# eniac/otti

Hardware: AMD Instinct MI355X
Metric: R1CS constraints/sec proved (Spartan NIZK) at 2^20 (higher is better)
Workload: dtype u256 (GF(l) / GF(2^255-19), 8 x u32 limbs)

## Files before the change

otti_amd/csrc/device.h:

```cpp
#pragma once
#include <hip/hip_runtime.h>
#include <vector>
#include <functional>
#include <cstddef>
#include <chrono>
#include "spartan.h"
#include "mail.h"
#include "msm_plan.h"

namespace otti {

#define OTTI_HIP(expr) ::otti::hip_check((expr), #expr, __FILE__, __LINE__)
void hip_check(hipError_t e, const char *what, const char *file, int line);
struct OutOfDeviceMemory : Error { using Error::Error; };
struct TailTimeout : Error { using Error::Error; };

template <class T> struct DevBuf {
    T *p = nullptr; size_t n = 0;
    DevBuf() {}
    explicit DevBuf(size_t count) { alloc(count); }
    DevBuf(const DevBuf &) = delete; DevBuf &operator=(const DevBuf &) = delete;
    DevBuf(DevBuf &&o) noexcept : p(o.p), n(o.n) { o.p = nullptr; o.n = 0; }
    DevBuf &operator=(DevBuf &&o) noexcept { if (this != &o) { release(); p = o.p; n = o.n; o.p = nullptr; o.n = 0; } return *this; }
    ~DevBuf() { release(); }
    void alloc(size_t count) { release(); if (count) OTTI_HIP(hipMalloc((void **)&p, count * sizeof(T))); n = count; }
    void release() { if (p) (void)hipFree(p); p = nullptr; n = 0; }
};

struct DCsr3 { const uint32_t *ptr[3]; const uint32_t *idx[3]; const Fr *val[3]; const int32_t *small[3]; };
struct DeviceCsrSet {
    DevBuf<uint32_t> ptr[3], idx[3]; DevBuf<Fr> val[3];
    DevBuf<int32_t> small[3];
    bool use_small = false;
    DevBuf<uint32_t> heavy;
    DevBuf<uint32_t> seg_row, seg_no, seg_begin;
    size_t rows = 0, n_heavy = 0, n_seg = 0;
    double avg_row = 0.0;
    bool quad() const { return avg_row >= 3.0; }
    DCsr3 view() const { DCsr3 v; for (int k = 0; k < 3; k++) { v.ptr[k] = ptr[k].p; v.idx[k] = idx[k].p; v.val[k] = val[k].p; v.small[k] = small[k].p; } return v; }
};
struct DeviceInstance { DeviceCsrSet by_row, by_col; size_t nnz = 0; };
struct DeviceShard { int rank = 0, world = 1; DeviceCsrSet by_row, by_col; };

struct DeviceGens {
    DevBuf<TabEntry> table; int c = 0, W = 0; size_t E = 0, nbases = 0;
    double build_ms[2] = {0, 0};
    const TabEntry *entry0(size_t base) const { return table.p + base * (size_t)W * E; }
};

struct Mailbox { Fr *partials; unsigned *counter; Fr *host_results; unsigned long long *host_flag; unsigned long long seq; int slot; int line_mail = 0;
                 Fr *dev_results; };

struct alignas(64) GoBox { unsigned long long seq, tag, pad[2]; Fr v[4]; unsigned long long timed_out, pad2[3]; };
static_assert(sizeof(GoBox) == 192 && offsetof(GoBox, v) == 32 && offsetof(GoBox, timed_out) == 160, "GoBox layout is read by hand-written loads");
constexpr int kGoCopies = 8;
constexpr size_t kGoCopyStride = 4096;
constexpr int kMsmMailRegions = 4;
struct PtFe;
bool msm_mail_sum(const MsmMail *m, int i0, int i1, unsigned long long want, PtFe &acc, unsigned max_spins, bool allow_ifma);
bool msm_mails_whole(const MsmMail *m, int n, unsigned long long want);
struct MsmPending { unsigned long long seq = 0, order = 0; int region = 0; uint32_t rows = 0, nchunks = 0; };
struct DevCtx;
struct MsmMailbox {
    MsmMail *host = nullptr, *dev = nullptr;
    MsmPending pending[kMsmMailRegions]; int pending_n = 0;
    unsigned long long launches = 0;
    unsigned long long read[8] = {0}; int read_next = 0;
    unsigned long long order = 0, h_pts_order = 0;
    bool host_sum(const DevCtx &c) const;
    void ensure(DevCtx &c);
    void queue(unsigned long long seq, uint32_t rows, uint32_t nchunks);
    MsmMail *region(int r) const { return host + (size_t)r * kMsmMailCap; }
};
struct TailMailbox { TailMail *host = nullptr, *dev = nullptr; void ensure(DevCtx &c); };
struct WaitLimits;
struct Armed { GoBox *host; GoBox *dev; unsigned long long want, deadline; int relay = 1, pollers = 1; };
constexpr unsigned long long kArmDeadlineTicks = 3000000000ull;
constexpr int kMaxBlocks = 2048;
constexpr size_t kArmMaxLen = 65536;

struct DevCtx {
    hipStream_t stream = nullptr;
    hipStream_t side = nullptr; hipEvent_t ev_side = nullptr;
    hipStream_t side_stream();
    int device = 0, num_cu = 256;
    DevBuf<Fr> partials;
    DevBuf<Fr> spmv_partial;
    DevBuf<Fr> results;
    Fr *h_results = nullptr;
    Fr *d_results_alias = nullptr;
    unsigned long long *h_flag = nullptr, *d_flag_alias = nullptr, seq = 0;
    DevBuf<unsigned> d_counter;
    DevBuf<unsigned long long> d_counts;
    DevBuf<unsigned long long> sat_bits;
    DevBuf<uint32_t> sat_rows; DevBuf<Fr> sat_abc;
    DevBuf<unsigned long long> diff_chunks;
    Mailbox next_mailbox(int slot);
    GoBox *h_go = nullptr, *d_go_alias = nullptr; DevBuf<GoBox> d_go; unsigned long long go_issued = 0, go_published = 0;
    unsigned long long arm_deadline = kArmDeadlineTicks;
    bool host_coherent = false;
    void reset_arrival_counters();
    hipEvent_t ev_order = nullptr;
    std::vector<struct RowSumSlot *> row_slots;
    TailMailbox tail_mail;
    template <class Pred, class OnLimit> void spin_until(Pred arrived, const WaitLimits &lim, std::chrono::steady_clock::time_point t0, OnLimit fail);
    void wait_tail(int n_groups, unsigned long long seq);
    void wait_tail_sums(int n_inst, int W, unsigned long long seq, Fr *sums);
    Armed arm_many(int count);
    bool armed_ok() const;
    Armed arm();
    void go(const Fr *v, int n);
    void go_abort();
    void wait_ticket(unsigned long long ticket);
    DevBuf<Pt> msm_keep;
    DevBuf<Pt> msm_partial, msm_final;
    Pt *h_pts = nullptr;
    size_t pending_host_encode = 0;
    uint8_t *h_points = nullptr;
    uint8_t *d_points_host = nullptr;
    DevBuf<uint8_t> d_points;
    size_t msm_partial_cap = 0, points_cap = 0;
    hipEvent_t ev0 = nullptr, ev1 = nullptr;
    static DevCtx &get();
    DevCtx() {} DevCtx(const DevCtx &) = delete; DevCtx &operator=(const DevCtx &) = delete;
    struct Scratch *scratch = nullptr;
    struct SnarkScratch *snark_scratch = nullptr;
    void sync();
    void wait_points(const MsmTicket &ticket);
    void encode_pending();
    Pt *d_pts_alias = nullptr; DevBuf<unsigned> d_counter2;
    MsmMailbox msm_mail;
    void msm_host_sum(const MsmPending &p);
    void ensure_points(size_t rows, size_t splits);
};
struct RowSumSlot { DevBuf<uint8_t> comp; DevBuf<Niels> pts; DevBuf<Fr> sc; DevBuf<Pt> out; DevBuf<unsigned> bad; bool busy = false; };
hipStream_t bulk_masked_stream();
struct ActiveProof { ActiveProof(); ~ActiveProof(); static int count(); };
constexpr int kResultSlots = 8192;

enum KClass { KC_MSM_ROWS = 0, KC_MSM_SMALL, KC_MSM_FINISH, KC_SC_CUBIC, KC_SC_QUAD, KC_SPMV, KC_EQ, KC_REDUCE, KC_BOUND, KC_BULLET, KC_OTHER,
              KC_PC_ROUND, KC_PROD_LAYER, KC_HASH_LAYER, KC_GATHER, KC_DOT_MANY ,
              KC_DECODE, KC_MSM_VAR , KC_SAT_CHECK , KC_COUNT };
struct KStats {
    bool on = false; unsigned mask = 0xffffffffu;
    std::vector<hipEvent_t> pool; std::vector<int> cls; size_t used = 0;
    double total_ms[KC_COUNT] = {0}; unsigned long long count[KC_COUNT] = {0};
    static KStats &get();
    int begin(DevCtx &c, int k);
    void end(DevCtx &c, int rec);
    void flush();
    void reset();
};
struct KScope { DevCtx &c; int rec; KScope(DevCtx &c_, int k) : c(c_), rec(KStats::get().begin(c_, k)) {} ~KScope() { KStats::get().end(c, rec); } };

enum WitFormat { WIT_CANONICAL32 = 0, WIT_MONTGOMERY32 = 1, WIT_I64 = 2, WIT_U64 = 3 };
inline size_t wit_elem_bytes(int format) { return format == WIT_I64 || format == WIT_U64 ? 8 : 32; }
struct DeviceWitness {
    DevBuf<Fr> z; std::vector<Fr> inputs;
    double small_fraction = 0.0;
    DeviceWitness(const Instance &I, int format, const void *src, size_t nvars, size_t stride, bool src_on_device, hipStream_t producer, const std::vector<Fr> &inputs);
    DeviceWitness(const Instance &I, const uint8_t *vars32, size_t nvars, const std::vector<Fr> &inputs) : DeviceWitness(I, WIT_CANONICAL32, vars32, nvars, 0, false, nullptr, inputs) {}
    void update(size_t first, int format, const void *src, size_t count, size_t stride, bool src_on_device, hipStream_t producer);
    void scatter(const uint64_t *idx, int format, const void *src, size_t count, size_t stride, bool on_device, hipStream_t producer);
    unsigned long long scatter_calls = 0, rows_patched = 0, terms_patched = 0;
    size_t assign(size_t first, int format, const void *src, size_t count, size_t stride, bool src_on_device, hipStream_t producer);
    size_t diff(size_t first, int format, const void *src, size_t count, size_t stride, bool src_on_device, hipStream_t producer, uint64_t *idx_out, size_t cap) const;
    unsigned long long assign_calls = 0, assign_changed = 0, assign_resums = 0;
    void set_inputs(const std::vector<Fr> &new_inputs);
    DevBuf<Pt> rows_kept; const char *rows_stream = nullptr; size_t rows_R = 0;
    Gens *rows_gens = nullptr;
    unsigned long long rows_resummed = 0;
    bool rows_kept_for(const Gens &g) const;
    void keep_rows(Gens &g);
    void drop_rows();
private:
    std::vector<Fr> set_up(DevCtx &c, const Instance &I, size_t nvars);
};
void ensure_device_objects(Instance &I, Gens &g);
void ensure_instance_device(Instance &I);
void ensure_gens_device(Gens &g);
void release_gens_device(Gens &g);
int device_window_bits(size_t nbases);
constexpr int kInstEvalSlot = 16;
void instance_evaluate_begin(Instance &I, const std::vector<Fr> &rx, const std::vector<Fr> &ry);
void instance_evaluate_finish(Fr out[3]);
void instance_evaluate_gpu(Instance &I, const std::vector<Fr> &rx, const std::vector<Fr> &ry, Fr out[3]);
class ShardComm;
std::vector<uint8_t> nizk_prove_resident(Instance &I, DeviceWitness &wit, Gens &g, const void *tlabel, size_t tlabel_len, const uint8_t *seed32,
                                         ProveTimings *tm, ShardComm *sh = nullptr);
struct R1csHooks { std::function<void(const std::vector<Fr> &)> on_rx, on_ry; std::function<void()> on_idle; };
void r1cs_prove_device(Instance &I, DeviceWitness &wit, Gens &g, Transcript &tr, RandomTape &tape, NizkProof &P, ProveTimings &T, ShardComm *sh, const R1csHooks *hooks = nullptr);
std::shared_ptr<DeviceShard> upload_instance_shard(const Instance &I, int rank, int world);
struct PeBufs { Fr *LZ, *Rv, *a, *s, *b2, *s2, *rows, *extras; };
DotProductProofLog dplog_prove_device(DevCtx &c, const DeviceGens &DG, const Gens &g, const PcView &v, const PeBufs &B, const Fr &LZ_blind, const Fr *y_known,
                                      const Fr &blind_y, CPoint &Cy_out, Transcript &tr, RandomTape &tape);
size_t dev_witness_ingest_from(DevCtx &c, int format, const void *src, size_t stride, size_t n, Fr *z, size_t dst_off, size_t *n_small = nullptr);
void dev_witness_scatter_check(DevCtx &c, int format, const void *src, size_t stride, const uint64_t *d_idx, size_t n, size_t V, Fr *conv,
                               size_t *bad_scalars, size_t *bad_indices);
void dev_witness_scatter_apply(DevCtx &c, const uint64_t *d_idx, const Fr *conv, size_t n, size_t V, Fr *z, Fr *delta);
struct WitDiff { size_t n_changed = 0, bad_scalars = 0, lo = 0, hi = 0; };
size_t dev_witness_diff_chunk();
WitDiff dev_witness_diff_count(DevCtx &c, int format, const void *src, size_t stride, size_t n, const Fr *z);
void dev_witness_diff_apply(DevCtx &c, int format, const void *src, size_t stride, size_t n, Fr *z, size_t first, size_t cap, uint64_t *d_idx, Fr *delta, bool write_z);
void dev_witness_rows_touched(DevCtx &c, const uint64_t *d_idx, size_t n, size_t R, uint64_t *h_rows);
void dev_gather_strided(DevCtx &c, const Fr *in, size_t stride, size_t offset, Fr *out, size_t n);

std::shared_ptr<DeviceInstance> upload_instance(const Instance &I);
std::shared_ptr<DeviceGens> build_device_gens(const Gens &g, int window_bits);

void dev_fr_op(DevCtx &c, int op, const Fr *a, const Fr *b, Fr *out, size_t n);
void dev_from_canonical(DevCtx &c, const Fr *in, Fr *out, size_t n);
void dev_to_canonical(DevCtx &c, const Fr *in, Fr *out, size_t n);
void dev_fill_zero(DevCtx &c, Fr *p, size_t n);
void dev_spmv3(DevCtx &c, const DeviceCsrSet &m, const Fr *x, Fr *out0, Fr *out1, Fr *out2, bool combine, const Fr coef[3]);
constexpr int kSatCountSlot = 24;
constexpr size_t kSatReportRows = 64;
struct SatReport { uint64_t n_unsat = 0; std::vector<uint64_t> rows; std::vector<uint8_t> abc96; float kernel_ms = 0; };
void dev_sat_pass(DevCtx &c, const DeviceCsrSet &m, const Fr *z, unsigned long long *bits);
uint64_t dev_sat_count(DevCtx &c);
SatReport dev_check_sat(DevCtx &c, DeviceInstance &d, const Fr *z, size_t max_rows, bool with_values);
void dev_eq_evals(DevCtx &c, const Fr *r_host, size_t ell, Fr *out, Fr *scratch );
void dev_eq_evals2(DevCtx &c, const Fr *r0_host, size_t ell0, Fr *out0, const Fr *r1_host, size_t ell1, Fr *out1, Fr *scratch);
unsigned long long dev_sc_cubic_eval(DevCtx &c, const Fr *A, const Fr *B, const Fr *C, const Fr *D, size_t len, int slot);
unsigned long long dev_sc_cubic_fold_eval(DevCtx &c, Fr *A, Fr *B, Fr *C, Fr *D, size_t len, const Fr &r, int slot);
struct EqSrc { const Fr *hi, *lo; int lo_bits;
               uint32_t stride = 1, offset = 0;
               int top_bit = -1; Fr top; };
void dev_eq_pyramid(DevCtx &c, const Fr *r_host, size_t n, Fr *out );
void dev_eq_pyramid2(DevCtx &c, const Fr *r0_host, size_t n0, Fr *out0, const Fr *r1_host, size_t n1, Fr *out1);
unsigned long long dev_sc_cubic3_eval(DevCtx &c, const Fr *B, const Fr *C, const Fr *D, size_t len, const EqSrc &E, int slot);
unsigned long long dev_sc_cubic3_fold_eval(DevCtx &c, Fr *B, Fr *C, Fr *D, size_t len, const Fr &r, const EqSrc &E, int slot);
unsigned long long dev_sc_cubic3_fold_eval_armed(DevCtx &c, Fr *B, Fr *C, Fr *D, size_t len, const EqSrc &E, int slot);
unsigned long long dev_sc_quad_fold_eval_armed(DevCtx &c, Fr *A, Fr *B, size_t len, int slot);
unsigned long long dev_sc_quad_eval(DevCtx &c, const Fr *A, const Fr *B, size_t len, int slot);
unsigned long long dev_sc_quad_fold_eval(DevCtx &c, Fr *A, Fr *B, size_t len, const Fr &r, int slot);
void dev_fold_top(DevCtx &c, Fr *Z, size_t len, const Fr &r);
void dev_fold_bot(DevCtx &c, const Fr *Z, Fr *out, size_t len, const Fr &r);
void dev_fetch(DevCtx &c, const Fr *src, int slot, size_t n);
struct MsmJob {
    const Fr *dense = nullptr; size_t n_dense = 0, rows = 0;
    const Fr *extra_s = nullptr; const uint32_t *extra_base = nullptr ; size_t n_extra = 0;
    int mode = MSM_COMPRESSED;
    const Pt *addend = nullptr;
    bool sparse = false;
    Pt *keep_dst = nullptr; bool force_bulk = false;
};
constexpr double kSparseWitness = 0.25;
MsmTicket dev_msm_rows(DevCtx &c, const DeviceGens &g, const MsmJob &job);
double dev_small_fraction(DevCtx &c, const Fr *z, size_t n);
void dev_msm_scatter(DevCtx &c, const DeviceGens &g, const uint64_t *d_idx, const Fr *d_s, size_t count, size_t R, Pt *rows, size_t L);
void dev_encode_points(DevCtx &c, const Pt *pts, size_t n, uint8_t *d_out32);
void dev_poly_bound(DevCtx &c, const Fr *Z, size_t L, size_t R, const Fr *Lv, Fr *out, Fr *scratch );
bool dev_poly_bound_chunks(DevCtx &c, const Fr *Z, size_t L, size_t R, const Fr *Lv_rest, size_t m, Fr *out, Fr *scratch );
void dev_dot(DevCtx &c, const Fr *a, const Fr *b, size_t n, int slot);
void dev_bullet_step(DevCtx &c, Fr *a, Fr *b, Fr *s, size_t R, size_t n_cur, bool fold_first, const Fr &u, const Fr &u_inv, Fr *rows, Fr *extra_out);
void dev_bullet_finish(DevCtx &c, Fr *a, Fr *b, Fr *s, size_t R, const Fr &u, const Fr &u_inv, const Fr &d, Fr *rows, int slot_a);
struct BulletRound {
    size_t R, n_cur; bool fold; Fr u, u_inv;
    const Fr *a_in, *b_in, *s_in; Fr *a_out, *b_out, *s_out;
    const Fr *extra_s; const uint32_t *extra_base; bool armed = false;
};
MsmTicket dev_bullet_round(DevCtx &c, const DeviceGens &g, const BulletRound &round);
void dev_decode_niels(DevCtx &c, const uint8_t *compressed_dev, size_t n, Niels *out, unsigned *bad);
int dev_msm_var(DevCtx &c, const Niels *pts, const Fr *scalars, size_t n, Pt *out, size_t out_cap, int *n_windows, int *n_splits);
double dev_madd_peak(DevCtx &c);
void dev_fr_to_lanes(hipStream_t st, const Fr *d_src, const Fr *factor, unsigned long long *d_lanes, size_t n);
double dev_fr_mul_peak(DevCtx &c);
void dev_scale(DevCtx &c, const Fr *in, const Fr &k, Fr *out, size_t n);
void dev_fill_one(DevCtx &c, Fr *p, size_t n);

}
```

otti_amd/csrc/k_sumcheck.hip:

```cpp
#include "kernels_common.h"

namespace otti {

struct FrArgs { Fr v[13]; };
struct EqJob { FrArgs r; int n; int pyramid; Fr *out; };
constexpr int kEqLow = 6, kEqTreeBlock = 256, kEqTreeGroups = 16;
__device__ __forceinline__ Fr eq_mul9(const Fr &x, const Fr &y) { return fr9_pack_lt2l(fr9_mul(fr9_unpack5(x), fr9_unpack(y))); }
__global__ __launch_bounds__(kEqTreeBlock) void k_eq_tree(EqJob j0, EqJob j1) {
    const EqJob &J = blockIdx.y ? j1 : j0;
    const int n = J.n, a = n < kEqLow ? n : kEqLow, b = n - a;
    __shared__ Fr sT[2 << kEqLow], sU[256];
    if (threadIdx.x == 0) { sT[0] = fr_one(); sU[0] = fr_one(); }
    __syncthreads();
    for (int s = 1; s <= (a > b ? a : b); s++) {
        const int half = 1 << (s - 1), t = (int)threadIdx.x;
        if (s <= a && t < half) { const Fr o = sT[half - 1 + t], hi = eq_mul9(o, J.r.v[n - s]); sT[2 * half - 1 + half + t] = hi; sT[2 * half - 1 + t] = fr_sub(o, hi); }
        if (s <= b && t >= 64 && t < 64 + half) { const int i = t - 64; const Fr o = sU[half - 1 + i], hi = eq_mul9(o, J.r.v[n - a - s]); sU[2 * half - 1 + half + i] = hi; sU[2 * half - 1 + i] = fr_sub(o, hi); }
        __syncthreads();
    }
    const size_t tid = blockIdx.x * (size_t)blockDim.x + threadIdx.x, nthr = (size_t)gridDim.x * blockDim.x, lowmask = ((size_t)1 << a) - 1;
    const Fr *Ta = sT + lowmask;
    if (J.pyramid) {
        const size_t small = ((size_t)2 << a) - 1, total = ((size_t)2 << n) - 1;
        if (blockIdx.x == 0) for (size_t g = threadIdx.x; g < small; g += blockDim.x) J.out[g] = sT[g];
        for (size_t g = small + tid; g < total; g += nthr) {
            const int k = 63 - __builtin_clzll((unsigned long long)(g + 1));
            const size_t i = g + 1 - ((size_t)1 << k);
            J.out[g] = eq_mul9(sU[((size_t)1 << (k - a)) - 1 + (i >> a)], Ta[i & lowmask]);
        }
    } else {
        const size_t total = (size_t)1 << n;
        const Fr *Ub = sU + (((size_t)1 << b) - 1);
        for (size_t i = tid; i < total; i += nthr) J.out[i] = b ? eq_mul9(Ub[i >> a], Ta[i & lowmask]) : Ta[i];
    }
}
static void launch_eq_tree(DevCtx &c, const Fr *r0, size_t n0, bool pyr0, Fr *out0, const Fr *r1, size_t n1, bool pyr1, Fr *out1) {
    if (n0 > 13 || n1 > 13) throw Error(OTTI_ERR_BAD_ARG, "eq table job over more than 13 variables");
    EqJob a, b;
    for (size_t i = 0; i < 13; i++) { a.r.v[i] = i < n0 ? r0[i] : fr_zero(); b.r.v[i] = (out1 && i < n1) ? r1[i] : fr_zero(); }
    a.n = (int)n0; a.pyramid = pyr0 ? 1 : 0; a.out = out0; b.n = out1 ? (int)n1 : 0; b.pyramid = pyr1 ? 1 : 0; b.out = out1;
    const size_t big = std::max(n0, out1 ? n1 : (size_t)0);
    const unsigned groups = big > (size_t)kEqLow ? (unsigned)std::min<size_t>(kEqTreeGroups, (((size_t)2 << big) + kEqTreeBlock - 1) / kEqTreeBlock) : 1u;
    hipLaunchKernelGGL(k_eq_tree, dim3(groups, out1 ? 2u : 1u), kEqTreeBlock, 0, c.stream, a, b);
}
__global__ __launch_bounds__(kBlock) void k_eq_expand(const Fr *__restrict__ hi, const Fr *__restrict__ lo, int lo_bits, Fr *__restrict__ out, size_t n_hi, size_t per) {
    const size_t j = blockIdx.x * (size_t)blockDim.x + threadIdx.x;
    const Fr9 l9 = fr9_unpack(lo[j]);
    const size_t h0 = (size_t)blockIdx.y * per, h1 = min(n_hi, h0 + per);
    for (size_t h = h0; h < h1; h++)
        out[(h << lo_bits) | j] = fr9_pack_lt2l(fr9_mul(fr9_unpack5(hi[h]), l9));
}
void dev_eq_evals2(DevCtx &c, const Fr *r0, size_t ell0, Fr *out0, const Fr *r1, size_t ell1, Fr *out1, Fr *scratch) {
    if (ell0 > 13 || ell1 > 13) { dev_eq_evals(c, r0, ell0, out0, scratch); dev_eq_evals(c, r1, ell1, out1, scratch); return; }
    KScope ks(c, KC_EQ);
    launch_eq_tree(c, r0, ell0, false, out0, r1, ell1, false, out1);
}
void dev_eq_evals(DevCtx &c, const Fr *r, size_t ell, Fr *out, Fr *scratch) {
    KScope ks(c, KC_EQ);
    if (ell <= 13) { launch_eq_tree(c, r, ell, false, out, nullptr, 0, false, nullptr); return; }
    const int lo_bits = 12, hi_bits = (int)ell - 12;
    if (hi_bits > 13) throw Error(OTTI_ERR_BAD_ARG, "eq table larger than 2^25");
    Fr *lo = scratch, *hi = scratch + 4096;
    launch_eq_tree(c, r + hi_bits, lo_bits, false, lo, r, (size_t)hi_bits, false, hi);
    const size_t n_hi = (size_t)1 << hi_bits, per = std::min<size_t>(16, std::max<size_t>(1, n_hi / 128));
    hipLaunchKernelGGL(k_eq_expand, dim3((unsigned)(((size_t)1 << lo_bits) / kBlock), (unsigned)((n_hi + per - 1) / per)), kBlock, 0, c.stream, hi, lo, lo_bits, out, n_hi, per);
}

__device__ __forceinline__ Pair load_pair(const Fr *T, size_t i, size_t half) { Pair p; p.lo = T[i]; p.hi = T[i + half]; return p; }
__device__ __forceinline__ Pair fold_pair(Fr *T, size_t i, size_t q, const Fr &r) {
    Fr a = T[i], b = T[i + q], c = T[i + 2 * q], d = T[i + 3 * q];
    Pair p; p.lo = fr_add(a, fr_mul(r, fr_sub(c, a))); p.hi = fr_add(b, fr_mul(r, fr_sub(d, b)));
    T[i] = p.lo; T[i + q] = p.hi;
    return p;
}
template <int K> __device__ __forceinline__ void store_partials(Fr (&acc)[K], Fr *partials) {
    block_reduce<K>(acc);
    if (threadIdx.x == 0) for (int k = 0; k < K; k++) partials[(size_t)blockIdx.x * K + k] = acc[k];
}
enum { POST_NONE = 0, POST_CUBIC3 = 1 };
template <int K, int kPost = POST_NONE> __device__ __forceinline__ void finish_in_kernel(Fr (&acc)[K], const Mailbox &mb) {
    block_reduce<K>(acc);
    if (gridDim.x > 1) {
        if (threadIdx.x == 0) for (int k = 0; k < K; k++) store_words_sc1(&mb.partials[(size_t)blockIdx.x * K + k], acc[k].v, 8);
        if (!arrive_and_check_last(mb.counter, gridDim.x)) return;
        for (int k = 0; k < K; k++) acc[k] = fr_zero();
        for (unsigned b = threadIdx.x; b < gridDim.x; b += blockDim.x)
            for (int k = 0; k < K; k++) { Fr t; load_words_sc1(t.v, &mb.partials[(size_t)b * K + k], 8); acc[k] = fr_add(acc[k], t); }
        block_reduce<K>(acc);
    }
    if (mb.line_mail && K <= 3) {
        __shared__ Fr s_line[3];
        if (threadIdx.x == 0) {
            if constexpr (kPost == POST_CUBIC3) quadratic_to_023(acc);
            for (int k = 0; k < 3; k++) { s_line[k] = k < K ? acc[k] : fr_zero(); if (k < K) mb.dev_results[mb.slot + k] = acc[k]; }
        }
        __syncthreads();
        if (threadIdx.x < 8) {
            typedef uint32_t u32x4 __attribute__((ext_vector_type(4)));
            const unsigned lane = threadIdx.x;
            u32x4 q = {0u, 0u, 0u, 0u};
            if (lane < 6) { const Fr &x = s_line[lane >> 1]; for (int i = 0; i < 4; i++) q[i] = x.v[4 * (lane & 1) + i]; }
            else if (lane == 6) { const unsigned long long tag = line_tag(mb.seq, s_line); q[0] = (uint32_t)mb.seq; q[1] = (uint32_t)(mb.seq >> 32); q[2] = (uint32_t)tag; q[3] = (uint32_t)(tag >> 32); }
            asm volatile("global_store_dwordx4 %0, %1, off sc0 sc1" :: "v"(reinterpret_cast<char *>(mb.host_results) + 16 * lane), "v"(q) : "memory");
        }
        return;
    }
    if (threadIdx.x == 0) {
        if constexpr (kPost == POST_CUBIC3) { static_assert(K == 3, "three totals"); quadratic_to_023(acc); }
        for (int k = 0; k < K; k++) { mb.dev_results[mb.slot + k] = acc[k]; mb.host_results[mb.slot + k] = acc[k]; }
        __threadfence_system();
        __hip_atomic_store(mb.host_flag, mb.seq, __ATOMIC_RELEASE, __HIP_MEMORY_SCOPE_SYSTEM);
    }
}
__device__ __forceinline__ void cubic4_accum9(Fr9 (&acc)[3], const Fr9 &a_lo5, const Fr9 &a_hi5, const Fr9 &b_lo, const Fr9 &b_hi, const Fr9 &c_lo5, const Fr9 &c_hi5,
                                              const Fr9 &d_lo, const Fr9 &d_hi) {
    acc[0] = fr9_add(acc[0], fr9_mul(a_lo5, fr9_sub_kl<4>(fr9_mul(b_lo, c_lo5), d_lo)));
    const Fr9 da5 = fr9_sub_kl<128>(a_hi5, a_lo5), db = fr9_sub_kl<4>(b_hi, b_lo), dc5 = fr9_sub_kl<128>(c_hi5, c_lo5), dd = fr9_sub_kl<4>(d_hi, d_lo);
    const Fr9 a2 = fr9_norm(fr9_add(a_hi5, da5)), b2 = fr9_norm(fr9_add(b_hi, db)), c2 = fr9_add(c_hi5, dc5), d2 = fr9_norm(fr9_add(d_hi, dd));
    acc[1] = fr9_add(acc[1], fr9_mul(a2, fr9_sub_kl<16>(fr9_mul(b2, c2), d2)));
    const Fr9 a3 = fr9_norm(fr9_add(a2, da5)), b3 = fr9_norm(fr9_add(b2, db)), c3 = fr9_norm(fr9_add(c2, dc5)), d3 = fr9_norm(fr9_add(d2, dd));
    acc[2] = fr9_add(acc[2], fr9_mul(a3, fr9_sub_kl<16>(fr9_mul(b3, c3), d3)));
}
__global__ __launch_bounds__(kBlock) void k_sc_cubic_eval(const Fr *A, const Fr *B, const Fr *C, const Fr *D, size_t half, Mailbox mb) {
    Fr9 acc[3] = {fr9_zero(), fr9_zero(), fr9_zero()}; unsigned n = 0;
    for (size_t i = blockIdx.x * (size_t)blockDim.x + threadIdx.x; i < half; i += (size_t)gridDim.x * blockDim.x) {
        const Fr a0 = A[i], a1 = A[i + half], b0 = B[i], b1 = B[i + half], c0 = C[i], c1 = C[i + half], d0 = D[i], d1 = D[i + half];
        __builtin_amdgcn_sched_barrier(0);
        cubic4_accum9(acc, fr9_unpack5(a0), fr9_unpack5(a1), fr9_unpack(b0), fr9_unpack(b1), fr9_unpack5(c0), fr9_unpack5(c1), fr9_unpack(d0), fr9_unpack(d1));
        if ((++n & 3u) == 0) acc9_carry(acc);
    }
    Fr tot[3]; acc9_canon<3>(tot, acc);
    finish_in_kernel<3>(tot, mb);
}
__global__ __launch_bounds__(kBlock) void k_sc_cubic_fold_eval(Fr *A, Fr *B, Fr *C, Fr *D, size_t q, Fr r, Mailbox mb) {
    const Fr9 r5 = fr9_unpack5(r);
    Fr9 acc[3] = {fr9_zero(), fr9_zero(), fr9_zero()}; unsigned n = 0;
    for (size_t i = blockIdx.x * (size_t)blockDim.x + threadIdx.x; i < q; i += (size_t)gridDim.x * blockDim.x) {
        const Fr a0 = A[i], a1 = A[i + q], a2 = A[i + 2 * q], a3 = A[i + 3 * q];
        const Fr b0 = B[i], b1 = B[i + q], b2 = B[i + 2 * q], b3 = B[i + 3 * q];
        __builtin_amdgcn_sched_barrier(0);
        Fr w0, w1;
        const Fr9 a_lo = fold9(a0, a2, r5, w0), a_hi = fold9(a1, a3, r5, w1); A[i] = w0; A[i + q] = w1;
        const Fr c0 = C[i], c1 = C[i + q], c2 = C[i + 2 * q], c3 = C[i + 3 * q];
        const Fr d0 = D[i], d1 = D[i + q], d2 = D[i + 2 * q], d3 = D[i + 3 * q];
        __builtin_amdgcn_sched_barrier(0);
        const Fr9 b_lo = fold9(b0, b2, r5, w0), b_hi = fold9(b1, b3, r5, w1); B[i] = w0; B[i + q] = w1;
        const Fr9 c_lo = fold9(c0, c2, r5, w0), c_hi = fold9(c1, c3, r5, w1); C[i] = w0; C[i + q] = w1;
        const Fr9 d_lo = fold9(d0, d2, r5, w0), d_hi = fold9(d1, d3, r5, w1); D[i] = w0; D[i + q] = w1;
        cubic4_accum9(acc, fr9_shl5(a_lo), fr9_shl5(a_hi), b_lo, b_hi, fr9_shl5(c_lo), fr9_shl5(c_hi), d_lo, d_hi);
        if ((++n & 3u) == 0) acc9_carry(acc);
    }
    Fr tot[3]; acc9_canon<3>(tot, acc);
    finish_in_kernel<3>(tot, mb);
}
__device__ __forceinline__ void cubic3_accum9(Fr9 (&acc)[3], const Fr9 &e5, const Fr9 &b_lo, const Fr9 &b_hi, const Fr9 &c_lo5, const Fr9 &c_hi5, const Fr9 &d_lo, const Fr9 &d_hi) {
    const Fr9 db = fr9_norm(fr9_sub_kl<4>(b_hi, b_lo));
    const Fr9 dc5 = fr9_sub_kl<128>(c_hi5, c_lo5);
    const Fr9 x0 = fr9_sub_kl<4>(fr9_mul(b_lo, c_lo5), d_lo);
    const Fr9 x1 = fr9_sub_kl<4>(fr9_mul(b_hi, c_hi5), d_hi);
    const Fr9 xi = fr9_mul(db, dc5);
    acc[0] = fr9_add(acc[0], fr9_mul(e5, x0));
    acc[1] = fr9_add(acc[1], fr9_mul(e5, x1));
    acc[2] = fr9_add(acc[2], fr9_mul(e5, xi));
}
__global__ __launch_bounds__(kBlock) void k_sc_cubic3_eval(const Fr *B, const Fr *C, const Fr *D, size_t half, EqSrc E, Mailbox mb) {
    Fr9 acc[3] = {fr9_zero(), fr9_zero(), fr9_zero()}; unsigned n = 0;
    for (size_t i = blockIdx.x * (size_t)blockDim.x + threadIdx.x; i < half; i += (size_t)gridDim.x * blockDim.x) {
        const Fr b0 = B[i], b1 = B[i + half], c0 = C[i], c1 = C[i + half], d0 = D[i], d1 = D[i + half];
        const Fr9 e5 = eq5_at(E, i);
        __builtin_amdgcn_sched_barrier(0);
        cubic3_accum9(acc, e5, fr9_unpack(b0), fr9_unpack(b1), fr9_unpack5(c0), fr9_unpack5(c1), fr9_unpack(d0), fr9_unpack(d1));
        if ((++n & 3u) == 0) acc9_carry(acc);
    }
    Fr tot[3]; acc9_canon<3>(tot, acc);
    finish_in_kernel<3, POST_CUBIC3>(tot, mb);
}
__global__ __launch_bounds__(kBlock) void k_sc_cubic3_fold_eval(Fr *B, Fr *C, Fr *D, size_t q, Fr r, EqSrc E, Mailbox mb, Armed go) {
    if (go.want) { Fr v[1]; if (!armed_fetch<1>(go, v)) return; r = v[0]; }
    const Fr9 r5 = fr9_unpack5(r);
    Fr9 acc[3] = {fr9_zero(), fr9_zero(), fr9_zero()}; unsigned n = 0;
    for (size_t i = blockIdx.x * (size_t)blockDim.x + threadIdx.x; i < q; i += (size_t)gridDim.x * blockDim.x) {
        const Fr b0 = B[i], b1 = B[i + q], b2 = B[i + 2 * q], b3 = B[i + 3 * q];
        const Fr c0 = C[i], c1 = C[i + q], c2 = C[i + 2 * q], c3 = C[i + 3 * q];
        __builtin_amdgcn_sched_barrier(0);
        Fr w0, w1;
        const Fr9 b_lo = fold9(b0, b2, r5, w0), b_hi = fold9(b1, b3, r5, w1); B[i] = w0; B[i + q] = w1;
        const Fr d0 = D[i], d1 = D[i + q], d2 = D[i + 2 * q], d3 = D[i + 3 * q];
        const Fr9 e5 = eq5_at(E, i);
        __builtin_amdgcn_sched_barrier(0);
        const Fr9 c_lo = fold9(c0, c2, r5, w0), c_hi = fold9(c1, c3, r5, w1); C[i] = w0; C[i + q] = w1;
        const Fr9 d_lo = fold9(d0, d2, r5, w0), d_hi = fold9(d1, d3, r5, w1); D[i] = w0; D[i + q] = w1;
        cubic3_accum9(acc, e5, b_lo, b_hi, fr9_shl5(c_lo), fr9_shl5(c_hi), d_lo, d_hi);
        if ((++n & 3u) == 0) acc9_carry(acc);
    }
    Fr tot[3]; acc9_canon<3>(tot, acc);
    finish_in_kernel<3, POST_CUBIC3>(tot, mb);
}
__device__ __forceinline__ void quad_accum9(Fr9 (&acc)[2], const Fr9 &a_lo, const Fr9 &a_hi, const Fr9 &b_lo5, const Fr9 &b_hi5) {
    acc[0] = fr9_add(acc[0], fr9_mul(a_lo, b_lo5));
    const Fr9 u = fr9_norm(fr9_sub_kl<4>(fr9_add(a_hi, a_hi), a_lo));
    const Fr9 v5 = fr9_sub_kl<128>(fr9_add(b_hi5, b_hi5), b_lo5);
    acc[1] = fr9_add(acc[1], fr9_mul(u, v5));
}
__global__ __launch_bounds__(kBlock) void k_sc_quad_eval(const Fr *A, const Fr *B, size_t half, Mailbox mb) {
    Fr9 acc[2] = {fr9_zero(), fr9_zero()}; unsigned n = 0;
    for (size_t i = blockIdx.x * (size_t)blockDim.x + threadIdx.x; i < half; i += (size_t)gridDim.x * blockDim.x) {
        const Fr a0 = A[i], a1 = A[i + half], b0 = B[i], b1 = B[i + half];
        __builtin_amdgcn_sched_barrier(0);
        quad_accum9(acc, fr9_unpack(a0), fr9_unpack(a1), fr9_unpack5(b0), fr9_unpack5(b1));
        if ((++n & 3u) == 0) { acc[0] = fr9_norm(acc[0]); acc[1] = fr9_norm(acc[1]); }
    }
    Fr tot[2]; acc9_canon<2>(tot, acc);
    finish_in_kernel<2>(tot, mb);
}
__global__ __launch_bounds__(kBlock) void k_sc_quad_fold_eval(Fr *A, Fr *B, size_t q, Fr r, Mailbox mb, Armed go) {
    if (go.want) { Fr v[1]; if (!armed_fetch<1>(go, v)) return; r = v[0]; }
    const Fr9 r5 = fr9_unpack5(r);
    Fr9 acc[2] = {fr9_zero(), fr9_zero()}; unsigned n = 0;
    for (size_t i = blockIdx.x * (size_t)blockDim.x + threadIdx.x; i < q; i += (size_t)gridDim.x * blockDim.x) {
        const Fr a0 = A[i], a1 = A[i + q], a2 = A[i + 2 * q], a3 = A[i + 3 * q];
        const Fr b0 = B[i], b1 = B[i + q], b2 = B[i + 2 * q], b3 = B[i + 3 * q];
        __builtin_amdgcn_sched_barrier(0);
        Fr w0, w1;
        const Fr9 a_lo = fold9(a0, a2, r5, w0), a_hi = fold9(a1, a3, r5, w1); A[i] = w0; A[i + q] = w1;
        const Fr9 b_lo = fold9(b0, b2, r5, w0), b_hi = fold9(b1, b3, r5, w1); B[i] = w0; B[i + q] = w1;
        quad_accum9(acc, a_lo, a_hi, fr9_shl5(b_lo), fr9_shl5(b_hi));
        if ((++n & 3u) == 0) { acc[0] = fr9_norm(acc[0]); acc[1] = fr9_norm(acc[1]); }
    }
    Fr tot[2]; acc9_canon<2>(tot, acc);
    finish_in_kernel<2>(tot, mb);
}
__global__ __launch_bounds__(kBlock) void k_fold_top(Fr *Z, size_t half, Fr r) {
    for (size_t i = blockIdx.x * (size_t)blockDim.x + threadIdx.x; i < half; i += (size_t)gridDim.x * blockDim.x) {
        Fr a = Z[i], b = Z[i + half]; Z[i] = fr_add(a, fr_mul(r, fr_sub(b, a)));
    }
}
__global__ __launch_bounds__(kBlock) void k_fold_bot(const Fr *Z, Fr *out, size_t half, Fr r) {
    for (size_t i = blockIdx.x * (size_t)blockDim.x + threadIdx.x; i < half; i += (size_t)gridDim.x * blockDim.x) {
        Fr a = Z[2 * i], b = Z[2 * i + 1]; out[i] = fr_add(a, fr_mul(r, fr_sub(b, a)));
    }
}
template <int K> static void finish_round(DevCtx &c, int nblocks, int slot) {
    { KScope ks(c, KC_REDUCE); hipLaunchKernelGGL(k_reduce_partials<K>, 1, kBlock, 0, c.stream, (const Fr *)c.partials.p, nblocks, c.results.p + slot); }
    dev_fetch(c, c.results.p + slot, slot, K);
}
static inline int sc_grid(size_t n) { return std::min(grid_for(n), n <= ((size_t)1 << 21) ? 512 : kMaxBlocks); }
unsigned long long dev_sc_cubic_eval(DevCtx &c, const Fr *A, const Fr *B, const Fr *C, const Fr *D, size_t len, int slot) {
    size_t half = len / 2; int g = sc_grid(half); Mailbox mb = c.next_mailbox(slot);
    KScope ks(c, KC_SC_CUBIC); hipLaunchKernelGGL(k_sc_cubic_eval, g, kBlock, 0, c.stream, A, B, C, D, half, mb);
    return mb.seq;
}
unsigned long long dev_sc_cubic_fold_eval(DevCtx &c, Fr *A, Fr *B, Fr *C, Fr *D, size_t len, const Fr &r, int slot) {
    if (len < 4) throw Error(OTTI_ERR_INTERNAL, "fold_eval needs len >= 4");
    size_t q = len / 4; int g = sc_grid(q); Mailbox mb = c.next_mailbox(slot);
    KScope ks(c, KC_SC_CUBIC); hipLaunchKernelGGL(k_sc_cubic_fold_eval, g, kBlock, 0, c.stream, A, B, C, D, q, r, mb);
    return mb.seq;
}
void dev_eq_pyramid(DevCtx &c, const Fr *r_host, size_t n, Fr *out) { dev_eq_pyramid2(c, r_host, n, out, nullptr, 0, nullptr); }
void dev_eq_pyramid2(DevCtx &c, const Fr *r0_host, size_t n0, Fr *out0, const Fr *r1_host, size_t n1, Fr *out1) {
    KScope ks(c, KC_EQ);
    launch_eq_tree(c, r0_host, n0, true, out0, r1_host, n1, true, out1);
}
unsigned long long dev_sc_cubic3_eval(DevCtx &c, const Fr *B, const Fr *C, const Fr *D, size_t len, const EqSrc &E, int slot) {
    size_t half = len / 2; int g = sc_grid(half); Mailbox mb = c.next_mailbox(slot);
    KScope ks(c, KC_SC_CUBIC); hipLaunchKernelGGL(k_sc_cubic3_eval, g, kBlock, 0, c.stream, B, C, D, half, E, mb);
    return mb.seq;
}
static unsigned long long cubic3_fold_eval(DevCtx &c, Fr *B, Fr *C, Fr *D, size_t len, const Fr *r, const EqSrc &E, int slot) {
    if (len < 4) throw Error(OTTI_ERR_INTERNAL, "fold_eval needs len >= 4");
    size_t q = len / 4; int g = sc_grid(q); Mailbox mb = c.next_mailbox(slot);
    const Armed go = r ? Armed{nullptr, nullptr, 0} : c.arm();
    KScope ks(c, KC_SC_CUBIC); hipLaunchKernelGGL(k_sc_cubic3_fold_eval, g, kBlock, 0, c.stream, B, C, D, q, r ? *r : fr_zero(), E, mb, go);
    return mb.seq;
}
unsigned long long dev_sc_cubic3_fold_eval(DevCtx &c, Fr *B, Fr *C, Fr *D, size_t len, const Fr &r, const EqSrc &E, int slot) { return cubic3_fold_eval(c, B, C, D, len, &r, E, slot); }
unsigned long long dev_sc_cubic3_fold_eval_armed(DevCtx &c, Fr *B, Fr *C, Fr *D, size_t len, const EqSrc &E, int slot) { return cubic3_fold_eval(c, B, C, D, len, nullptr, E, slot); }
unsigned long long dev_sc_quad_eval(DevCtx &c, const Fr *A, const Fr *B, size_t len, int slot) {
    size_t half = len / 2; int g = sc_grid(half); Mailbox mb = c.next_mailbox(slot);
    KScope ks(c, KC_SC_QUAD); hipLaunchKernelGGL(k_sc_quad_eval, g, kBlock, 0, c.stream, A, B, half, mb);
    return mb.seq;
}
static unsigned long long quad_fold_eval(DevCtx &c, Fr *A, Fr *B, size_t len, const Fr *r, int slot) {
    if (len < 4) throw Error(OTTI_ERR_INTERNAL, "fold_eval needs len >= 4");
    size_t q = len / 4; int g = sc_grid(q); Mailbox mb = c.next_mailbox(slot);
    const Armed go = r ? Armed{nullptr, nullptr, 0} : c.arm();
    KScope ks(c, KC_SC_QUAD); hipLaunchKernelGGL(k_sc_quad_fold_eval, g, kBlock, 0, c.stream, A, B, q, r ? *r : fr_zero(), mb, go);
    return mb.seq;
}
unsigned long long dev_sc_quad_fold_eval(DevCtx &c, Fr *A, Fr *B, size_t len, const Fr &r, int slot) { return quad_fold_eval(c, A, B, len, &r, slot); }
unsigned long long dev_sc_quad_fold_eval_armed(DevCtx &c, Fr *A, Fr *B, size_t len, int slot) { return quad_fold_eval(c, A, B, len, nullptr, slot); }
void dev_fold_top(DevCtx &c, Fr *Z, size_t len, const Fr &r) { size_t h = len / 2; if (h) hipLaunchKernelGGL(k_fold_top, grid_for(h), kBlock, 0, c.stream, Z, h, r); }
void dev_fold_bot(DevCtx &c, const Fr *Z, Fr *out, size_t len, const Fr &r) { size_t h = len / 2; if (h) hipLaunchKernelGGL(k_fold_bot, grid_for(h), kBlock, 0, c.stream, Z, out, h, r); }

__global__ __launch_bounds__(kBlock) void k_dot(const Fr *a, const Fr *b, size_t n, Fr *partials) {
    Fr acc[1] = {fr_zero()};
    for (size_t i = blockIdx.x * (size_t)blockDim.x + threadIdx.x; i < n; i += (size_t)gridDim.x * blockDim.x) acc[0] = fr_add(acc[0], fr_mul(a[i], b[i]));
    store_partials<1>(acc, partials);
}
void dev_dot(DevCtx &c, const Fr *a, const Fr *b, size_t n, int slot) {
    int g = grid_for(n);
    hipLaunchKernelGGL(k_dot, g, kBlock, 0, c.stream, a, b, n, c.partials.p);
    finish_round<1>(c, g, slot);
}

template <int K> __device__ __forceinline__ Fr lanes_sum(Fr acc, int lane, int lanes, int cols) {
    __shared__ Fr sm[K][kBlock];
    if (lanes > 1) {
        sm[0][threadIdx.x] = acc;
        __syncthreads();
        for (int s = lanes >> 1; s >= 1; s >>= 1) {
            if (lane < s) { acc = fr_add(acc, sm[0][threadIdx.x + s * cols]); sm[0][threadIdx.x] = acc; }
            __syncthreads();
        }
    }
    return acc;
}
__global__ __launch_bounds__(kBlock) void k_poly_bound_slab(const Fr *Z, size_t L, size_t R, const Fr *Lv, size_t rows_per_slab, Fr *scratch, size_t lv_mask, int lanes_log2) {
    const int lanes = 1 << lanes_log2, cols = kBlock >> lanes_log2, lane = (int)threadIdx.x / cols, cj = (int)threadIdx.x % cols;
    const size_t j = blockIdx.x * (size_t)cols + cj;
    const size_t i0 = blockIdx.y * rows_per_slab, i1 = min(L, i0 + rows_per_slab);
    Fr acc = fr_zero();
    if (j < R) for (size_t i = i0 + lane; i < i1; i += lanes) acc = fr_add(acc, fr_mul(Lv[i & lv_mask], Z[i * R + j]));
    acc = lanes_sum<1>(acc, lane, lanes, cols);
    if (lane == 0 && j < R) scratch[(size_t)blockIdx.y * R + j] = acc;
}
constexpr int kColsumLanesLog2 = 3;
__global__ __launch_bounds__(kBlock) void k_colsum(const Fr *scratch, size_t slabs, size_t R, Fr *out) {
    const int lanes = 1 << kColsumLanesLog2, cols = kBlock >> kColsumLanesLog2, lane = (int)threadIdx.x / cols, cj = (int)threadIdx.x % cols;
    const size_t j = blockIdx.x * (size_t)cols + cj;
    Fr acc = fr_zero();
    if (j < R) for (size_t s = lane; s < slabs; s += lanes) acc = fr_add(acc, scratch[s * R + j]);
    acc = lanes_sum<1>(acc, lane, lanes, cols);
    if (lane == 0 && j < R) out[j] = acc;
}
static int bound_lanes_log2(size_t R, size_t slabs, size_t rps) {
    int lg = 0;
    while (lg < 2 && ((size_t)2 << lg) * 2 <= rps && ((R + (kBlock >> (lg + 1)) - 1) / (kBlock >> (lg + 1))) * slabs <= 2048) lg++;
    return lg;
}
void dev_poly_bound(DevCtx &c, const Fr *Z, size_t L, size_t R, const Fr *Lv, Fr *out, Fr *scratch) {
    size_t slabs = std::min<size_t>(L, 64), rps = (L + slabs - 1) / slabs;
    KScope ks(c, KC_BOUND);
    const int ll = bound_lanes_log2(R, slabs, rps); const size_t cols = (size_t)kBlock >> ll, ccols = (size_t)kBlock >> kColsumLanesLog2;
    dim3 grid((unsigned)((R + cols - 1) / cols), (unsigned)slabs);
    hipLaunchKernelGGL(k_poly_bound_slab, grid, kBlock, 0, c.stream, Z, L, R, Lv, rps, scratch, ~(size_t)0, ll);
    hipLaunchKernelGGL(k_colsum, (unsigned)((R + ccols - 1) / ccols), kBlock, 0, c.stream, (const Fr *)scratch, slabs, R, out);
}
__global__ __launch_bounds__(kBlock) void k_colsum_groups(const Fr *scratch, size_t group, size_t R, Fr *out) {
    size_t j = blockIdx.x * (size_t)blockDim.x + threadIdx.x;
    if (j >= R) return;
    const Fr *base = scratch + (size_t)blockIdx.y * group * R;
    Fr acc = base[j];
    for (size_t s = 1; s < group; s++) acc = fr_add(acc, base[s * R + j]);
    out[(size_t)blockIdx.y * R + j] = acc;
}
bool dev_poly_bound_chunks(DevCtx &c, const Fr *Z, size_t L, size_t R, const Fr *Lv_rest, size_t m, Fr *out, Fr *scratch) {
    const size_t slabs = std::min<size_t>(L, 64), rps = (L + slabs - 1) / slabs;
    if (!m || (m & (m - 1)) || m > L || L % m || m % rps || slabs * rps != L) return false;
    KScope ks(c, KC_BOUND);
    const int ll = bound_lanes_log2(R, slabs, rps); const size_t cols = (size_t)kBlock >> ll;
    dim3 grid((unsigned)((R + cols - 1) / cols), (unsigned)slabs);
    hipLaunchKernelGGL(k_poly_bound_slab, grid, kBlock, 0, c.stream, Z, L, R, Lv_rest, rps, scratch, m - 1, ll);
    hipLaunchKernelGGL(k_colsum_groups, dim3((unsigned)((R + kBlock - 1) / kBlock), (unsigned)(L / m)), kBlock, 0, c.stream, (const Fr *)scratch, m / rps, R, out);
    return true;
}

}
```

Baseline: 379.2 million.

## Size sumcheck grids from occupancy and deal block reductions across wave lanes

Replaces the fixed sumcheck grid heuristic with a planner that caps workgroups by measured per-CU residency, balances items per thread, and limits armed launches to a fixed count. Also replaces the per-sum block reduction with a dealt reduction that splits two or three accumulators across lane halves and quarters, so each shuffle tree reduces one value instead of K. The aim is less tail imbalance and fewer shuffles in the reduction epilogue, at the cost of extra code and an occupancy query on first use.

Result: faster. 390.8 million, median of 6 (+3.1%).

```diff
diff --git a/otti_amd/csrc/device.h b/otti_amd/csrc/device.h
--- a/otti_amd/csrc/device.h
+++ b/otti_amd/csrc/device.h
@@ -7,6 +7,7 @@
 #include "spartan.h"
 #include "mail.h"
 #include "msm_plan.h"
+#include "sc_plan.h"
 
 namespace otti {
 
@@ -234,6 +235,7 @@
 unsigned long long dev_sc_quad_fold_eval_armed(DevCtx &c, Fr *A, Fr *B, size_t len, int slot);
 unsigned long long dev_sc_quad_eval(DevCtx &c, const Fr *A, const Fr *B, size_t len, int slot);
 unsigned long long dev_sc_quad_fold_eval(DevCtx &c, Fr *A, Fr *B, size_t len, const Fr &r, int slot);
+const ScCaps &sc_caps(DevCtx &c);
 void dev_fold_top(DevCtx &c, Fr *Z, size_t len, const Fr &r);
 void dev_fold_bot(DevCtx &c, const Fr *Z, Fr *out, size_t len, const Fr &r);
 void dev_fetch(DevCtx &c, const Fr *src, int slot, size_t n);
diff --git a/otti_amd/csrc/k_sumcheck.hip b/otti_amd/csrc/k_sumcheck.hip
--- a/otti_amd/csrc/k_sumcheck.hip
+++ b/otti_amd/csrc/k_sumcheck.hip
@@ -78,15 +78,44 @@
     if (threadIdx.x == 0) for (int k = 0; k < K; k++) partials[(size_t)blockIdx.x * K + k] = acc[k];
 }
 enum { POST_NONE = 0, POST_CUBIC3 = 1 };
+template <int K> __device__ __forceinline__ void block_reduce_dealt(Fr (&acc)[K]) {
+    static_assert(K == 2 || K == 3, "two or three sums");
+    __shared__ Fr sm[K][16];
+    const int lane = threadIdx.x & 63, wave = threadIdx.x >> 6, nw = blockDim.x >> 6;
+    const bool up = (lane & 32) != 0, up2 = (lane & 16) != 0;
+    Fr one;
+    int mine;
+    if constexpr (K == 2) {
+        const Fr got = shfl_xor_fr(up ? acc[0] : acc[1], 32);
+        one = fr_add(up ? acc[1] : acc[0], got); mine = up ? 1 : 0;
+    } else {
+        const Fr z = fr_zero();
+        const Fr got0 = shfl_xor_fr(up ? acc[0] : acc[2], 32), got1 = shfl_xor_fr(up ? acc[1] : z, 32);
+        const Fr two0 = fr_add(up ? acc[2] : acc[0], got0), two1 = up ? z : fr_add(acc[1], got1);
+        const Fr got = shfl_xor_fr(up2 ? two0 : two1, 16);
+        one = fr_add(up2 ? two1 : two0, got); mine = (up ? 2 : 0) + (up2 ? 1 : 0);
+    }
+#pragma unroll
+    for (int off = K == 2 ? 16 : 8; off >= 1; off >>= 1) one = fr_add(one, shfl_xor_fr(one, off));
+    __syncthreads();
+    if ((lane & (K == 2 ? 31 : 15)) == 0 && mine < K) sm[mine][wave] = one;
+    __syncthreads();
+    if (threadIdx.x < 64) {
+        Fr t = fr_zero();
+        if (lane < K) { t = sm[lane][0]; for (int w = 1; w < nw; w++) t = fr_add(t, sm[lane][w]); }
+#pragma unroll
+        for (int k = 0; k < K; k++) acc[k] = shfl_xor_fr(t, k);
+    }
+}
 template <int K, int kPost = POST_NONE> __device__ __forceinline__ void finish_in_kernel(Fr (&acc)[K], const Mailbox &mb) {
-    block_reduce<K>(acc);
+    block_reduce_dealt<K>(acc);
     if (gridDim.x > 1) {
         if (threadIdx.x == 0) for (int k = 0; k < K; k++) store_words_sc1(&mb.partials[(size_t)blockIdx.x * K + k], acc[k].v, 8);
         if (!arrive_and_check_last(mb.counter, gridDim.x)) return;
         for (int k = 0; k < K; k++) acc[k] = fr_zero();
         for (unsigned b = threadIdx.x; b < gridDim.x; b += blockDim.x)
             for (int k = 0; k < K; k++) { Fr t; load_words_sc1(t.v, &mb.partials[(size_t)b * K + k], 8); acc[k] = fr_add(acc[k], t); }
-        block_reduce<K>(acc);
+        block_reduce_dealt<K>(acc);
     }
     if (mb.line_mail && K <= 3) {
         __shared__ Fr s_line[3];
@@ -244,15 +273,33 @@
     { KScope ks(c, KC_REDUCE); hipLaunchKernelGGL(k_reduce_partials<K>, 1, kBlock, 0, c.stream, (const Fr *)c.partials.p, nblocks, c.results.p + slot); }
     dev_fetch(c, c.results.p + slot, slot, K);
 }
-static inline int sc_grid(size_t n) { return std::min(grid_for(n), n <= ((size_t)1 << 21) ? 512 : kMaxBlocks); }
+template <class Kern> static unsigned resident_workgroups(const DevCtx &c, Kern kern) {
+    int per_cu = 0;
+    OTTI_HIP(hipOccupancyMaxActiveBlocksPerMultiprocessor(&per_cu, kern, kBlock, 0));
+    return (unsigned)std::max(1, per_cu) * (unsigned)std::max(1, c.num_cu);
+}
+const ScCaps &sc_caps(DevCtx &c) {
+    static std::once_flag once; static ScCaps caps;
+    std::call_once(once, [&] {
+        caps.num_cu = (unsigned)std::max(1, c.num_cu);
+        caps.resident[(int)ScKind::cubic3_eval] = resident_workgroups(c, k_sc_cubic3_eval);
+        caps.resident[(int)ScKind::cubic3_fold] = resident_workgroups(c, k_sc_cubic3_fold_eval);
+        caps.resident[(int)ScKind::quad_eval] = resident_workgroups(c, k_sc_quad_eval);
+        caps.resident[(int)ScKind::quad_fold] = resident_workgroups(c, k_sc_quad_fold_eval);
+        caps.resident[(int)ScKind::cubic4_eval] = resident_workgroups(c, k_sc_cubic_eval);
+        caps.resident[(int)ScKind::cubic4_fold] = resident_workgroups(c, k_sc_cubic_fold_eval);
+    });
+    return caps;
+}
+static_assert(kScThreads == kBlock && kScMaxWorkgroups == (unsigned)kMaxBlocks && (size_t)kScArmedWorkgroups * kBlock * 4 == kArmMaxLen, "sc_plan.h restates device.h");
 unsigned long long dev_sc_cubic_eval(DevCtx &c, const Fr *A, const Fr *B, const Fr *C, const Fr *D, size_t len, int slot) {
-    size_t half = len / 2; int g = sc_grid(half); Mailbox mb = c.next_mailbox(slot);
+    size_t half = len / 2; const unsigned g = sc_plan(ScKind::cubic4_eval, len, false, sc_caps(c)).workgroups; Mailbox mb = c.next_mailbox(slot);
     KScope ks(c, KC_SC_CUBIC); hipLaunchKernelGGL(k_sc_cubic_eval, g, kBlock, 0, c.stream, A, B, C, D, half, mb);
     return mb.seq;
 }
 unsigned long long dev_sc_cubic_fold_eval(DevCtx &c, Fr *A, Fr *B, Fr *C, Fr *D, size_t len, const Fr &r, int slot) {
     if (len < 4) throw Error(OTTI_ERR_INTERNAL, "fold_eval needs len >= 4");
-    size_t q = len / 4; int g = sc_grid(q); Mailbox mb = c.next_mailbox(slot);
+    size_t q = len / 4; const unsigned g = sc_plan(ScKind::cubic4_fold, len, false, sc_caps(c)).workgroups; Mailbox mb = c.next_mailbox(slot);
     KScope ks(c, KC_SC_CUBIC); hipLaunchKernelGGL(k_sc_cubic_fold_eval, g, kBlock, 0, c.stream, A, B, C, D, q, r, mb);
     return mb.seq;
 }
@@ -262,29 +309,29 @@
     launch_eq_tree(c, r0_host, n0, true, out0, r1_host, n1, true, out1);
 }
 unsigned long long dev_sc_cubic3_eval(DevCtx &c, const Fr *B, const Fr *C, const Fr *D, size_t len, const EqSrc &E, int slot) {
-    size_t half = len / 2; int g = sc_grid(half); Mailbox mb = c.next_mailbox(slot);
+    size_t half = len / 2; const unsigned g = sc_plan(ScKind::cubic3_eval, len, false, sc_caps(c)).workgroups; Mailbox mb = c.next_mailbox(slot);
     KScope ks(c, KC_SC_CUBIC); hipLaunchKernelGGL(k_sc_cubic3_eval, g, kBlock, 0, c.stream, B, C, D, half, E, mb);
     return mb.seq;
 }
 static unsigned long long cubic3_fold_eval(DevCtx &c, Fr *B, Fr *C, Fr *D, size_t len, const Fr *r, const EqSrc &E, int slot) {
     if (len < 4) throw Error(OTTI_ERR_INTERNAL, "fold_eval needs len >= 4");
-    size_t q = len / 4; int g = sc_grid(q); Mailbox mb = c.next_mailbox(slot);
+    size_t q = len / 4; const ScPlan p = sc_plan(ScKind::cubic3_fold, len, !r, sc_caps(c)); Mailbox mb = c.next_mailbox(slot);
     const Armed go = r ? Armed{nullptr, nullptr, 0} : c.arm();
-    KScope ks(c, KC_SC_CUBIC); hipLaunchKernelGGL(k_sc_cubic3_fold_eval, g, kBlock, 0, c.stream, B, C, D, q, r ? *r : fr_zero(), E, mb, go);
+    KScope ks(c, KC_SC_CUBIC); hipLaunchKernelGGL(k_sc_cubic3_fold_eval, p.workgroups, kBlock, 0, c.stream, B, C, D, q, r ? *r : fr_zero(), E, mb, go);
     return mb.seq;
 }
 unsigned long long dev_sc_cubic3_fold_eval(DevCtx &c, Fr *B, Fr *C, Fr *D, size_t len, const Fr &r, const EqSrc &E, int slot) { return cubic3_fold_eval(c, B, C, D, len, &r, E, slot); }
 unsigned long long dev_sc_cubic3_fold_eval_armed(DevCtx &c, Fr *B, Fr *C, Fr *D, size_t len, const EqSrc &E, int slot) { return cubic3_fold_eval(c, B, C, D, len, nullptr, E, slot); }
 unsigned long long dev_sc_quad_eval(DevCtx &c, const Fr *A, const Fr *B, size_t len, int slot) {
-    size_t half = len / 2; int g = sc_grid(half); Mailbox mb = c.next_mailbox(slot);
+    size_t half = len / 2; const unsigned g = sc_plan(ScKind::quad_eval, len, false, sc_caps(c)).workgroups; Mailbox mb = c.next_mailbox(slot);
     KScope ks(c, KC_SC_QUAD); hipLaunchKernelGGL(k_sc_quad_eval, g, kBlock, 0, c.stream, A, B, half, mb);
     return mb.seq;
 }
 static unsigned long long quad_fold_eval(DevCtx &c, Fr *A, Fr *B, size_t len, const Fr *r, int slot) {
     if (len < 4) throw Error(OTTI_ERR_INTERNAL, "fold_eval needs len >= 4");
-    size_t q = len / 4; int g = sc_grid(q); Mailbox mb = c.next_mailbox(slot);
+    size_t q = len / 4; const ScPlan p = sc_plan(ScKind::quad_fold, len, !r, sc_caps(c)); Mailbox mb = c.next_mailbox(slot);
     const Armed go = r ? Armed{nullptr, nullptr, 0} : c.arm();
-    KScope ks(c, KC_SC_QUAD); hipLaunchKernelGGL(k_sc_quad_fold_eval, g, kBlock, 0, c.stream, A, B, q, r ? *r : fr_zero(), mb, go);
+    KScope ks(c, KC_SC_QUAD); hipLaunchKernelGGL(k_sc_quad_fold_eval, p.workgroups, kBlock, 0, c.stream, A, B, q, r ? *r : fr_zero(), mb, go);
     return mb.seq;
 }
 unsigned long long dev_sc_quad_fold_eval(DevCtx &c, Fr *A, Fr *B, size_t len, const Fr &r, int slot) { return quad_fold_eval(c, A, B, len, &r, slot); }
diff --git a/otti_amd/csrc/sc_plan.h b/otti_amd/csrc/sc_plan.h
--- /dev/null
+++ b/otti_amd/csrc/sc_plan.h
@@ -0,0 +1,37 @@
+#pragma once
+#include <algorithm>
+#include <cstddef>
+
+namespace otti {
+
+constexpr int kScThreads = 256;
+constexpr unsigned kScArmedWorkgroups = 64;
+constexpr unsigned kScMaxWorkgroups = 2048;
+
+enum class ScKind { cubic3_eval = 0, cubic3_fold = 1, quad_eval = 2, quad_fold = 3, cubic4_eval = 4, cubic4_fold = 5 };
+constexpr int kScKinds = 6;
+
+constexpr unsigned kScWorkgroupsPerCu = 2;
+constexpr size_t kScWideItems = (size_t)1 << 21;
+
+struct ScCaps {
+    unsigned num_cu = 256;
+    unsigned resident[kScKinds] = {512, 512, 512, 512, 512, 512};
+};
+struct ScPlan { unsigned workgroups; size_t items, items_per_thread; };
+
+inline size_t sc_ceil_div(size_t a, size_t b) { return (a + b - 1) / b; }
+
+inline ScPlan sc_plan(ScKind kind, size_t len, bool armed, const ScCaps &caps) {
+    const bool fold = ((int)kind & 1) != 0;
+    ScPlan p;
+    p.items = std::max<size_t>(1, fold ? len / 4 : len / 2);
+    unsigned cap = p.items > kScWideItems ? kScMaxWorkgroups : std::min(caps.resident[(int)kind], kScWorkgroupsPerCu * caps.num_cu);
+    cap = std::max(1u, std::min(cap, armed ? kScArmedWorkgroups : kScMaxWorkgroups));
+    const size_t need = sc_ceil_div(p.items, kScThreads);
+    p.workgroups = need <= cap ? (unsigned)need : (unsigned)sc_ceil_div(need, sc_ceil_div(need, cap));
+    p.items_per_thread = sc_ceil_div(p.items, (size_t)p.workgroups * kScThreads);
+    return p;
+}
+
+}
```
